# mitschabaude/msm-zprize

Measured on AMD Instinct MI355X. Metric: Mpoint-adds/s (ms per MSM in ms_per_step), higher is better.
Workload: dtype u32 limbs (28-bit lazy Montgomery, i64 accumulate)

## Files before the change

### msm_zprize_amd/_native.py

```python
import ctypes as C
import os

HERE = os.path.dirname(os.path.abspath(__file__))
LIB_PATH = os.environ.get("MSMZ_LIB") or os.path.join(HERE, "libmsmz.so")

MSMZ_N_STAGES = 8
STAGE_NAMES = ["digits", "scan", "scatter", "plan", "accumulate", "reduce", "final", "total"]


class MsmzOpts(C.Structure):
    _fields_ = [("c", C.c_int32), ("glv", C.c_int32), ("safe", C.c_int32), ("buckets", C.c_int32),
                ("timing", C.c_int32), ("reserved", C.c_int32 * 3)]


class MsmzLog(C.Structure):
    _fields_ = [("stage_ms", C.c_float * MSMZ_N_STAGES), ("c", C.c_int32), ("K", C.c_int32), ("rounds", C.c_int32),
                ("glv", C.c_int32), ("n_entries", C.c_uint64), ("n_pairs", C.c_uint64), ("max_bucket", C.c_uint32),
                ("scatter_launches", C.c_uint32), ("scatter_kernel_ms", C.c_float), ("batch_add_ms", C.c_float * 32)]


MSMZ_SRC_DEVICE, MSMZ_SRC_MONTGOMERY, MSMZ_SRC_DEFAULT_STREAM = 1, 2, 4
MSMZ_SRC_COMPRESSED, MSMZ_SRC_SIGN_PARITY = 8, 16
MSMZ_ERR_POINT = 7

# ... 76 lines not shown
                ("bins", C.c_void_p), ("packed", C.c_void_p)]


TEST_SORT_GEOM = ["c", "K", "Keff", "L", "nb", "fb", "fbt", "ncb", "ncbt", "nbins", "sbins", "fbins", "fine_top", "spread",
                  "fold_shift", "fold_rows", "F", "mbits", "idx_bits", "cspec", "two_level", "tiles", "sbits", "endo_delta"]


EXPORTS = {
    "msmz_create": (C.c_int, [C.POINTER(C.c_void_p), C.c_int, C.POINTER(C.c_int), C.c_int]),
    "msmz_destroy": (None, [C.c_void_p]),
    "msmz_strerror": (C.c_char_p, [C.c_int]),
    "msmz_curve_fe_bytes": (C.c_int, [C.c_int]),
    "msmz_ctx_fe_bytes": (C.c_int, [C.c_void_p]),
    "msmz_ctx_n_devices": (C.c_int, [C.c_void_p]),
    "msmz_upload_points": (C.c_int, [C.c_void_p, C.c_char_p, C.c_char_p, C.c_uint64, C.POINTER(C.c_uint64)]),
    "msmz_upload_scalars": (C.c_int, [C.c_void_p, C.c_char_p, C.c_uint64, C.POINTER(C.c_uint64)]),
    "msmz_import_scalars": (C.c_int, [C.c_void_p, C.POINTER(MsmzSrc), C.c_uint64, C.POINTER(C.c_uint64)]),
    "msmz_import_scalars_into": (C.c_int, [C.c_void_p, C.c_uint64, C.c_uint64, C.POINTER(MsmzSrc), C.c_uint64]),
    "msmz_alloc_scalars": (C.c_int, [C.c_void_p, C.c_uint64, C.POINTER(C.c_uint64)]),
    "msmz_import_points": (C.c_int, [C.c_void_p, C.POINTER(MsmzSrc), C.c_uint64, C.POINTER(C.c_uint64)]),
    "msmz_random_points": (C.c_int, [C.c_void_p, C.c_uint64, C.c_uint64, C.POINTER(C.c_uint64)]),
    "msmz_random_scalars": (C.c_int, [C.c_void_p, C.c_uint64, C.c_uint64, C.POINTER(C.c_uint64)]),
    "msmz_download_points": (C.c_int, [C.c_void_p, C.c_uint64, C.c_uint64, C.c_uint64, C.c_char_p, C.c_char_p]),
    "msmz_download_points_compressed": (C.c_int, [C.c_void_p, C.c_uint64, C.c_uint64, C.c_uint64, C.c_char_p, C.c_char_p,
                                                  C.c_uint32]),
    "msmz_download_scalars": (C.c_int, [C.c_void_p, C.c_uint64, C.c_uint64, C.c_uint64, C.c_char_p]),
    "msmz_free": (C.c_int, [C.c_void_p, C.c_uint64]),
    "msmz_msm": (C.c_int, [C.c_void_p, C.c_uint64, C.c_char_p, C.c_uint64, C.POINTER(MsmzOpts), C.c_char_p,
                           C.POINTER(C.c_int), C.POINTER(MsmzLog)]),
    "msmz_msm_resident": (C.c_int, [C.c_void_p, C.c_uint64, C.c_uint64, C.c_uint64, C.POINTER(MsmzOpts), C.c_char_p,
                                    C.POINTER(C.c_int), C.POINTER(MsmzLog)]),
    "msmz_msm_batch": (C.c_int, [C.c_void_p, C.c_uint64, C.c_char_p, C.c_uint64, C.c_uint32, C.POINTER(MsmzOpts),
                                 C.c_char_p, C.POINTER(C.c_int), C.POINTER(MsmzLog)]),
    "msmz_msm_batch_resident": (C.c_int, [C.c_void_p, C.c_uint64, C.c_uint64, C.c_uint64, C.c_uint32,
                                          C.POINTER(MsmzOpts), C.c_char_p, C.POINTER(C.c_int), C.POINTER(MsmzLog)]),
    "msmz_msm_segments": (C.c_int, [C.c_void_p, C.c_uint64, C.c_uint64, C.POINTER(MsmzSegment), C.c_uint32,
                                    C.POINTER(MsmzOpts), C.c_char_p, C.POINTER(C.c_int), C.POINTER(MsmzLog)]),
    "msmz_precompute_points": (C.c_int, [C.c_void_p, C.c_uint64, C.c_uint64, C.POINTER(MsmzOpts), C.c_uint32,
                                         C.POINTER(C.c_uint64)]),
    "msmz_precomputed_info": (C.c_int, [C.c_void_p, C.c_uint64, C.POINTER(C.c_int32), C.POINTER(C.c_int32),
                                        C.POINTER(C.c_uint32), C.POINTER(C.c_uint32), C.POINTER(C.c_uint64)]),
    "msmz_precomputed_scalar_bits": (C.c_int, [C.c_void_p, C.c_uint64, C.POINTER(C.c_int32)]),
    "msmz_check_points": (C.c_int, [C.c_void_p, C.c_uint64, C.c_uint64, C.c_uint64, C.c_uint32,
                                    C.POINTER(MsmzCheckResult), C.c_char_p]),
    "msmz_points_mul": (C.c_int, [C.c_void_p, C.POINTER(MsmzMul), C.c_uint64, C.POINTER(C.c_uint64)]),
    "msmz_points_mul_opts": (C.c_int, [C.c_void_p, C.POINTER(MsmzMul), C.c_uint64, C.POINTER(MsmzMulOpts),
                                       C.POINTER(C.c_uint64)]),
    "msmz_scalars_combine": (C.c_int, [C.c_void_p, C.POINTER(MsmzScalarTerm), C.POINTER(MsmzScalarTerm), C.c_uint64,
                                       C.c_uint64, C.POINTER(C.c_uint64)]),
    "msmz_scalars_dot": (C.c_int, [C.c_void_p, C.c_uint64, C.c_uint64, C.c_uint64, C.c_uint64, C.c_uint64, C.c_char_p]),
    "msmz_scalars_powers": (C.c_int, [C.c_void_p, C.c_char_p, C.c_char_p, C.c_uint64, C.POINTER(C.c_uint64)]),
    "msmz_scalars_recurrence": (C.c_int, [C.c_void_p, C.POINTER(MsmzScalarRec), C.c_uint64, C.c_uint64,
                                          C.POINTER(C.c_uint64), C.c_char_p]),
    "msmz_scalars_inverse": (C.c_int, [C.c_void_p, C.c_uint64, C.c_uint64, C.c_uint64, C.c_uint64, C.POINTER(C.c_uint64),
                                       C.POINTER(C.c_uint64)]),
    "msmz_scalars_ntt": (C.c_int, [C.c_void_p, C.POINTER(MsmzNtt), C.c_uint64, C.POINTER(C.c_uint64)]),
    "msmz_scalars_root_of_unity": (C.c_int, [C.c_int, C.c_uint32, C.c_char_p]),
    "msmz_point_add": (C.c_int, [C.c_int, C.c_char_p, C.c_int, C.c_char_p, C.c_int, C.c_char_p, C.POINTER(C.c_int)]),
    "msmz_test_set_glv_bits": (C.c_int, [C.c_void_p, C.c_int]),
    "msmz_test_retries": (C.c_int, [C.c_void_p]),
    "msmz_test_set_limits": (C.c_int, [C.c_void_p, C.c_uint64, C.c_uint64]),
    "msmz_test_passes": (C.c_int, [C.c_void_p, C.POINTER(C.c_uint64), C.POINTER(C.c_uint64)]),
    "msmz_test_scalar_dot_geometry": (None, [C.POINTER(C.c_uint32), C.POINTER(C.c_uint32)]),
    "msmz_test_scalar_scan_geometry": (None, [C.POINTER(C.c_uint32), C.POINTER(C.c_uint32), C.POINTER(C.c_uint32)]),
    "msmz_test_ntt_plan": (C.c_int, [C.c_int, C.c_uint32, C.POINTER(C.c_uint32), C.POINTER(C.c_uint32)]),
    "msmz_test_ntt_geometry": (None, [C.POINTER(C.c_uint32)]),
    "msmz_test_field": (C.c_int, [C.c_void_p, C.c_int, C.c_char_p, C.c_char_p, C.c_uint64, C.c_char_p]),
    "msmz_test_field_limbs": (C.c_int, [C.c_void_p, C.c_int, C.c_void_p, C.c_void_p, C.c_uint64, C.c_void_p,
                                        C.c_char_p]),
    "msmz_test_field_rows": (C.c_int, [C.c_void_p, C.c_int, C.c_void_p, C.c_void_p, C.c_uint64, C.c_uint32, C.c_void_p,
                                       C.c_char_p]),
    "msmz_test_glv": (C.c_int, [C.c_void_p, C.c_char_p, C.c_uint64, C.c_char_p, C.c_char_p, C.c_char_p]),
    "msmz_test_digits": (C.c_int, [C.c_void_p, C.c_char_p, C.c_uint64, C.c_int, C.c_int, C.c_int, C.c_void_p]),
    "msmz_test_sort": (C.c_int, [C.c_void_p, C.c_char_p, C.c_uint64, C.c_int, C.c_int, C.c_int, C.c_void_p, C.c_void_p,
                                 C.c_uint64, C.c_void_p, C.c_uint64]),
    "msmz_test_sort_ex": (C.c_int, [C.c_void_p, C.POINTER(MsmzTestSortArgs)]),
    "msmz_test_point_raw": (C.c_int, [C.c_void_p, C.c_int, C.c_char_p, C.c_char_p, C.c_char_p, C.c_uint64, C.c_int,
                                      C.c_char_p]),
    "msmz_test_point": (C.c_int, [C.c_void_p, C.c_int, C.c_char_p, C.c_char_p, C.c_char_p, C.c_char_p, C.c_uint64,
                                  C.c_char_p]),
    "msmz_test_batch_add": (C.c_int, [C.c_void_p, C.c_int, C.c_int, C.c_char_p, C.c_char_p, C.c_uint64, C.c_char_p,
                                      C.c_char_p, C.c_uint64, C.c_void_p, C.c_uint64, C.c_uint64, C.c_char_p,
                                      C.POINTER(C.c_uint32)]),
    "msmz_test_reduce": (C.c_int, [C.c_void_p, C.POINTER(MsmzTestReduceArgs)]),
    "msmz_test_plan": (C.c_int, [C.c_void_p, C.POINTER(MsmzTestPlanArgs)]),
}

_lib = None


class MsmzError(RuntimeError):
    def __init__(self, status, where):
        self.status = status
        msg = lib().msmz_strerror(status).decode() if _lib is not None else "?"
        super().__init__(f"{where}: msmz status {status} ({msg})")


def lib():
    global _lib
    if _lib is None:
        if not os.path.exists(LIB_PATH):
            raise RuntimeError(f"{LIB_PATH} is missing: run `python -m msm_zprize_amd.build` "
                               "(the MSM has no CPU fallback)")
        l = C.CDLL(LIB_PATH)
        for name, (res, args) in EXPORTS.items():
            fn = getattr(l, name)
            fn.restype = res
            fn.argtypes = args
        _lib = l
    return _lib


def check(status, where):
    if status != 0:
        raise MsmzError(status, where)
```

### msm_zprize_amd/csrc/batch_kernels.h

```cpp
#pragma once

namespace msmz {

#ifndef MSMZ_BATCH_BMAX
#define MSMZ_BATCH_BMAX 16
#endif
#ifdef MSMZ_EXP_NOMUL
#define BM_MUL(r, a, b) fe_add(r, a, b)
#define BM_SQR(r, a) fe_add(r, a, a)
#else
#define BM_MUL(r, a, b) fe_mul(r, a, b)
#define BM_SQR(r, a) fe_sqr(r, a)
#endif
enum { PK_NONE = 0, PK_ADD = 1, PK_DBL = 2, PK_TAKE_A = 3, PK_TAKE_B = 4, PK_INF = 5 };

template <class F, int T, bool SAFE, int OCC, int BMAX>
__global__ void __launch_bounds__(T, OCC) k_batch_add(uint32_t* slots, const uint32_t* points, const uint2* dsc,
                                                      uint32_t out_base, uint32_t total, int B, MsmMeta* meta) {
  __shared__ int32_t tree[F::N * T];
  __shared__ int32_t s_prev[F::N * T];
  __shared__ uint8_t s_kind[SAFE ? BMAX * T : 1];
  constexpr int N = F::N;
  const uint32_t block_base = blockIdx.x * (uint32_t)(T * B);
#ifdef MSMZ_TRACE
// ... 14 lines not shown
#pragma unroll 1
  for (int i = 0; i < B; i++) {
    const uint32_t t = block_base + (uint32_t)i * T + threadIdx.x;
    uint32_t kind = PK_NONE;
    uint2 dd = dnext;
    if (i + 1 < B && t + (uint32_t)T < total) dnext = dsc[t + (uint32_t)T];
    if (t < total) {
#if defined(MSMZ_EXP_LOCALMEM) || defined(MSMZ_EXP_LOCAL_FWD)
      dd.x = LOC_ORIG | (t & 4095u);
      dd.y = LOC_ORIG | ((t + 1u) & 4095u);
#endif
      Fe<F> d;
      kind = PK_ADD;
      if constexpr (SAFE && SlotFmt<F>::PACKED) {
        Fe<F> x1, x2;
        const uint32_t oa = load_operand_x_or<F>(x1, dd.x, slots, points);
        const uint32_t ob = load_operand_x_or<F>(x2, dd.y, slots, points);
        fe_sub(d, x2, x1);
        if (oa == 0 || ob == 0 || fe_is_zero(d)) {
          Affine<F> p1, p2;
          const bool infA = load_operand<F, true>(p1, dd.x, slots, points);
          const bool infB = load_operand<F, true>(p2, dd.y, slots, points);
          if (infA) {
            kind = infB ? PK_INF : PK_TAKE_B;
          } else if (infB) {
            kind = PK_TAKE_A;
          } else if (fe_is_zero(d)) {
            Fe<F> num;
            fe_sub(num, p2.y, p1.y);
            if (fe_is_zero(num) && !fe_is_zero(p1.y)) {
              kind = PK_DBL;
              fe_add(d, p2.y, p2.y);
            } else {
              kind = PK_INF;
            }
          }
        }
      } else if constexpr (SAFE) {
        Affine<F> p1, p2;
        const bool infA = load_operand<F, true>(p1, dd.x, slots, points);
        const bool infB = load_operand<F, true>(p2, dd.y, slots, points);
        Fe<F> num;
        fe_sub(d, p2.x, p1.x);
        fe_sub(num, p2.y, p1.y);
        if (infA) {
          kind = infB ? PK_INF : PK_TAKE_B;
        } else if (infB) {
          kind = PK_TAKE_A;
        } else if (fe_is_zero(d)) {
          if (fe_is_zero(num) && !fe_is_zero(p1.y)) {
            kind = PK_DBL;
            fe_add(d, p2.y, p2.y);
          } else {
            kind = PK_INF;
          }
        }
      } else {
        Fe<F> x1, x2;
        load_operand_x<F>(x1, dd.x, slots, points);
        load_operand_x<F>(x2, dd.y, slots, points);
        fe_sub(d, x2, x1);
      }
      if (kind == PK_ADD || kind == PK_DBL) {
        if (i == ilast) {
#pragma unroll
          for (int j = 0; j < N; j++) s_prev[j * T + threadIdx.x] = prefix.l[j];
        } else if (i > 0) {
#if defined(MSMZ_EXP_LOCALMEM) || defined(MSMZ_EXP_LOCAL_Z)
          slot_store_mulout<F>(slots + slot_offset<F>(blockIdx.x * 64u + (t & 63u)), prefix);
#else
          slot_store_mulout<F>(slots + slot_offset<F>(out_base + t), prefix);
#endif
        }
        Fe<F> np;
        BM_MUL(np, prefix, d);
        prefix = np;
      }
    }
    if (SAFE) s_kind[i * T + threadIdx.x] = (uint8_t)kind;
  }

  MSMZ_STAMP(trace, 1);
  __builtin_amdgcn_s_setprio(3);
  Fe<F> run;
  {
    Fe<F> partner, node;
#pragma unroll
    for (int j = 0; j < N; j++) partner.l[j] = __shfl_xor(prefix.l[j], 1, 64);
    fe_mul(node, prefix, partner);
    if ((threadIdx.x & 1) == 0) {
#pragma unroll
      for (int j = 0; j < N; j++) tree[j * T + (threadIdx.x >> 1)] = node.l[j];
    }
  }
  __syncthreads();
  int lvl_off = 0;
#pragma unroll 1
  for (int width = T >> 2; width >= 1; width >>= 1) {
    const int child_off = lvl_off;
    lvl_off += width * 2;
    if ((int)threadIdx.x < width) {
      Fe<F> x, y, z;
#pragma unroll
      for (int j = 0; j < N; j++) {
        x.l[j] = tree[j * T + child_off + 2 * threadIdx.x];
        y.l[j] = tree[j * T + child_off + 2 * threadIdx.x + 1];
      }
      fe_mul(z, x, y);
#pragma unroll
      for (int j = 0; j < N; j++) tree[j * T + lvl_off + threadIdx.x] = z.l[j];
    }
    __syncthreads();
  }
  MSMZ_STAMP(trace, 2);
  if (threadIdx.x < 64) {
    Fe<F> root, inv;
#pragma unroll
    for (int j = 0; j < N; j++) root.l[j] = tree[j * T + lvl_off];
#ifdef MSMZ_EXP_NOINV
    const bool ok = true;
    inv = root;
#else
    const bool ok = fe_inverse_wave(inv, root);
#endif
    if (threadIdx.x == 0) {
      if (!ok) atomicOr(&meta->error, 1u);
#pragma unroll
      for (int j = 0; j < N; j++) tree[j * T + lvl_off] = inv.l[j];
    }
  }
  __syncthreads();
  MSMZ_STAMP(trace, 3);
#pragma unroll 1
  for (int width = 1; width <= T >> 2; width <<= 1) {
    const int parent_off = lvl_off;
    lvl_off -= width * 2;
    Fe<F> ci;
    const bool mine = (int)threadIdx.x < 2 * width;
    if (mine) {
      Fe<F> pi, sib;
#pragma unroll
      for (int j = 0; j < N; j++) {
        pi.l[j] = tree[j * T + parent_off + (threadIdx.x >> 1)];
        sib.l[j] = tree[j * T + lvl_off + (threadIdx.x ^ 1)];
      }
      fe_mul(ci, pi, sib);
    }
    __syncthreads();
    if (mine) {
#pragma unroll
      for (int j = 0; j < N; j++) tree[j * T + lvl_off + threadIdx.x] = ci.l[j];
    }
    __syncthreads();
  }
  {
    Fe<F> partner, ninv;
#pragma unroll
    for (int j = 0; j < N; j++) {
      partner.l[j] = __shfl_xor(prefix.l[j], 1, 64);
      ninv.l[j] = tree[j * T + (threadIdx.x >> 1)];
    }
    fe_mul(run, ninv, partner);
  }

  MSMZ_STAMP(trace, 4);
  __builtin_amdgcn_s_setprio(0);
  {
    const uint32_t tl = block_base + (uint32_t)(B - 1) * T + threadIdx.x;
    if (tl < total) dnext = dsc[tl];
  }
#pragma unroll 1
  for (int i = B - 1; i >= 0; i--) {
    const uint32_t t = block_base + (uint32_t)i * T + threadIdx.x;
    uint2 dd = dnext;
    if (i > 0 && t - (uint32_t)T < total) dnext = dsc[t - (uint32_t)T];
    if (t >= total) continue;
    const uint32_t kind = SAFE ? s_kind[i * T + threadIdx.x] : (uint32_t)PK_ADD;
#if defined(MSMZ_EXP_LOCALMEM) || defined(MSMZ_EXP_LOCAL_BWD)
    dd.x = LOC_ORIG | (t & 4095u);
    dd.y = LOC_ORIG | ((t + 1u) & 4095u);
#endif
#if defined(MSMZ_EXP_LOCALMEM) || defined(MSMZ_EXP_LOCAL_Z)
    uint32_t* out = slots + slot_offset<F>(blockIdx.x * 64u + (t & 63u));
#else
    uint32_t* out = slots + slot_offset<F>(out_base + t);
#endif
    if (kind == PK_ADD || kind == PK_DBL) {
      Affine<F> p2;
      load_operand<F, false>(p2, dd.y, slots, points);
      Fe<F> z, mm, ms, d, tt, s12, num;
      if (i == ilast) {
#pragma unroll
        for (int j = 0; j < N; j++) z.l[j] = s_prev[j * T + threadIdx.x];
      } else if (i > 0) {
        slot_load_fe<F>(z, out);
      } else {
        fe_set_const<F>(z, F::ONE);
      }
      if (kind == PK_ADD) {
        Affine<F> p1;
        load_operand<F, false>(p1, dd.x, slots, points);
        fe_sub(d, p2.x, p1.x);
        fe_sub(num, p2.y, p1.y);
        fe_add(s12, p2.x, p1.x);
      } else {
        fe_add(d, p2.y, p2.y);
        fe_add(s12, p2.x, p2.x);
        Fe<F> xx;
        fe_sqr(xx, p2.x);
        fe_add(num, xx, xx);
        fe_add(num, num, xx);
        fe_carry(num);
      }
      BM_MUL(tt, z, run);
      BM_MUL(mm, num, tt);
      BM_MUL(tt, run, d);
      run = tt;
      BM_SQR(ms, mm);
      Affine<F> res;
      fe_sub(res.x, ms, s12);
      fe_sub(tt, p2.x, res.x);
      fe_carry(tt);
      BM_MUL(ms, mm, tt);
      fe_sub(res.y, ms, p2.y);
      slot_store_point<F>(out, res, false);
    } else if (kind == PK_TAKE_A || kind == PK_TAKE_B) {
      Affine<F> p;
      load_operand<F, false>(p, kind == PK_TAKE_A ? dd.x : dd.y, slots, points);
      slot_store_point<F>(out, p, false);
    } else {
      Affine<F> dummy;
      fe_zero(dummy.x);
      fe_zero(dummy.y);
      slot_store_point<F>(out, dummy, true);
    }
  }
  MSMZ_STAMP(trace, 5);
}

}
```

### msm_zprize_amd/csrc/instantiate.h

```cpp
#pragma once
#include "check_kernels.h"
#include "gen_kernels.h"
#include "import_kernels.h"
#include "kernels.h"
#include "mul_kernels.h"
#include "ntt_kernels.h"
#include "scalar_kernels.h"
#include "scan_kernels.h"
#include "test_kernels.h"

#if !defined(MSMZ_CURVE) || MSMZ_CURVE == 0
#define MSMZ_W0(X) X(Bls377Fp, Bls377Fr)
#else
#define MSMZ_W0(X)
#endif
#if !defined(MSMZ_CURVE) || MSMZ_CURVE == 1
#define MSMZ_W1(X) X(PallasFp, PallasFr)
#else
#define MSMZ_W1(X)
#endif
#if !defined(MSMZ_CURVE) || MSMZ_CURVE == 2
#define MSMZ_W2(X) X(Bls381Fp, Bls381Fr)
#else
#define MSMZ_W2(X)
// ... 33 lines not shown
                                                uint32_t, uint32_t);                                             \
  PFX template __global__ void k_pairsum<P>(uint32_t*, const uint32_t*, uint32_t);                               \
  PFX template __global__ void k_fill_neutral<P>(uint32_t*, uint32_t);                                           \
  PFX template __global__ void k_bucket_sums<P>(uint32_t*, const uint32_t*, const uint32_t*, uint32_t);          \
  PFX template __global__ void k_reduce2d_partial_acc<P>(uint32_t*, const uint32_t*, const uint32_t*, R2Geom, uint32_t); \
  PFX template __global__ void k_pairsum_x4<P>(uint32_t*, const uint32_t*, uint32_t);                            \
  PFX template __global__ void k_bucket_accumulate<P>(uint32_t*, const uint32_t*, const uint32_t*,               \
                                                      const uint32_t*, const uint32_t*, uint32_t, uint32_t, int);

#define MSMZ_INST_REDUCE(F, Fr, PFX)                                                                              \
  PFX template __global__ void k_reduce2d_partial<F>(uint32_t*, const uint32_t*, const uint32_t*, const uint4*,   \
                                                     R2Geom, uint32_t);                                          \
  PFX template __global__ void k_reduce_affine_finish<F>(uint32_t*, uint32_t*, const uint32_t*, const uint32_t*,  \
                                                         const uint2*, const uint4*, F2Geom);                     \
  MSMZ_INST_POLICY(WeierPolicy<F>, PFX)

#define MSMZ_INST_REDUCE_TE(F, Fr, PFX) MSMZ_INST_POLICY(TePolicy<F>, PFX)

#define MSMZ_INST_TEST(F, Fr, P, PFX)                                                                             \
  PFX template __global__ void k_test_field<F>(uint32_t*, const uint32_t*, const uint32_t*, uint32_t, int, uint32_t*); \
  PFX template __global__ void k_test_field_limbs<F>(int32_t*, uint32_t*, const int32_t*, const int32_t*, uint32_t,  \
                                                      int, uint32_t*);                                            \
  PFX template __global__ void k_test_field_rows<F>(int32_t*, uint32_t*, const int32_t*, const int32_t*, uint32_t,   \
                                                     int, uint32_t);                                              \
  PFX template __global__ void k_test_glv<Fr>(uint32_t*, uint32_t*, uint8_t*, const uint32_t*, uint32_t);         \
  PFX template __global__ void k_test_digits<Fr, false>(uint32_t*, const uint32_t*, uint32_t, int, int);          \
  PFX template __global__ void k_test_point<P>(uint32_t*, const uint32_t*, const uint32_t*, const uint8_t*,   \
                                                   const uint8_t*, uint32_t, int);                                \
  PFX template __global__ void k_test_point_raw<P>(uint32_t*, const uint32_t*, const uint32_t*, const uint8_t*, \
                                                       uint32_t, int, int);                                       \
  PFX template __global__ void k_test_accs_in<P>(uint32_t*, const uint32_t*, const uint8_t*, const uint32_t*, \
                                                     uint32_t, uint32_t*);                                        \
  PFX template __global__ void k_test_accs_out<P>(uint32_t*, const uint32_t*, uint32_t);

#define MSMZ_INST_SORT(Fr, PFX, GLV, C, SEG)                                                                      \
  PFX template __global__ void k_hist<Fr, GLV, C, SEG>(uint32_t*, uint16_t*, uint32_t*, MsmMeta*, const uint32_t*, SortGeom, uint32_t, const SegDesc*); \
  PFX template __global__ void k_coarse<Fr, GLV, C, SEG>(uint32_t*, const uint32_t*, const uint32_t*, const uint16_t*, const uint32_t*, SortGeom, uint32_t, const SegDesc*);

#define MSMZ_INST_SCAN(Fr, AM, HB, PFX)                                                                           \
  PFX template __global__ void k_scalars_rec_tile<Fr, AM, HB>(uint32_t*, uint32_t*, const uint32_t*, const uint32_t*, FrConst, uint32_t, uint32_t, uint32_t*); \
  PFX template __global__ void k_scalars_rec_apply<Fr, AM, HB>(uint32_t*, const uint32_t*, const uint32_t*, FrConst, const uint32_t*, uint32_t, uint32_t);

#define MSMZ_INST_SCALAR(Fr, PFX)                                                                                 \
  PFX template __global__ void k_digits<Fr, false>(uint32_t*, uint32_t*, MsmMeta*, const uint32_t*, uint32_t, int, int, int, int); \
  MSMZ_SORT_INSTANCES(MSMZ_INST_SORT, Fr, PFX)                                                                    \
  PFX template __global__ void k_check_scalars<Fr>(uint32_t*, const uint32_t*, uint32_t);                         \
  PFX template __global__ void k_gen_scalars<Fr>(uint32_t*, uint32_t, uint64_t, GenMap);                          \
  PFX template __global__ void k_import_scalars<Fr>(uint32_t*, const uint8_t*, uint64_t, int, uint32_t, int, uint32_t*); \
  PFX template __global__ void k_scalars_combine<Fr>(uint32_t*, ScalarTerm, ScalarTerm, uint32_t, uint32_t*);     \
  PFX template __global__ void k_scalars_dot<Fr>(uint32_t*, const uint32_t*, const uint32_t*, uint32_t, uint32_t*); \
  PFX template __global__ void k_scalars_dot_fold<Fr>(uint32_t*, const uint32_t*, uint32_t, int);                 \
  PFX template __global__ void k_scalars_powers<Fr>(uint32_t*, FrConst, FrPowTable, uint32_t, GenMap);                \
  MSMZ_INST_SCAN(Fr, SREC_A_NONE, true, PFX)                                                                      \
  MSMZ_INST_SCAN(Fr, SREC_A_BROADCAST, false, PFX)                                                                \
  MSMZ_INST_SCAN(Fr, SREC_A_BROADCAST, true, PFX)                                                                 \
  MSMZ_INST_SCAN(Fr, SREC_A_RESIDENT, false, PFX)                                                                 \
  MSMZ_INST_SCAN(Fr, SREC_A_RESIDENT, true, PFX)                                                                  \
  PFX template __global__ void k_scalars_rec_carry<Fr, false, true>(uint32_t*, uint32_t*, const uint32_t*, const uint32_t*, FrConst, uint32_t); \
  PFX template __global__ void k_scalars_rec_carry<Fr, true, false>(uint32_t*, uint32_t*, const uint32_t*, const uint32_t*, FrConst, uint32_t); \
  PFX template __global__ void k_scalars_rec_carry<Fr, true, true>(uint32_t*, uint32_t*, const uint32_t*, const uint32_t*, FrConst, uint32_t); \
  PFX template __global__ void k_scalars_inverse<Fr>(uint32_t*, const uint32_t*, uint32_t, uint32_t*);         \
  PFX template __global__ void k_ntt_pass<Fr>(NttArgs);

#define MSMZ_INST_MISC_P(F, Fr, P, PFX)                                                                           \
  PFX template __global__ void k_points_to_resident<P>(uint32_t*, const uint32_t*, const uint8_t*, uint32_t, int, uint32_t*); \
  PFX template __global__ void k_points_from_resident<P>(uint32_t*, const uint32_t*, uint32_t);                   \
  PFX template __global__ void k_import_points<P>(uint32_t*, const uint8_t*, uint64_t, const uint8_t*, uint32_t, int, int, uint32_t*); \
  PFX template __global__ void k_import_points_compressed<P>(uint32_t*, const uint8_t*, uint64_t, const uint8_t*, uint32_t, int, int, uint32_t*); \
  PFX template __global__ void k_points_compress<P>(uint32_t*, uint8_t*, const uint32_t*, uint32_t, int);         \
  PFX template __global__ void k_check_curve<P>(uint8_t*, CheckResult*, const uint32_t*, uint32_t, uint32_t);     \
  PFX template __global__ void k_check_subgroup<P, Fr>(uint8_t*, CheckResult*, const uint32_t*, uint32_t, uint32_t); \
  PFX template __global__ void k_points_mul<P, Fr, false>(uint32_t*, const uint32_t*, const uint32_t*, MulScalar, const uint32_t*, uint32_t, int, int, uint32_t*); \
  PFX template __global__ void k_points_mul<P, Fr, true>(uint32_t*, const uint32_t*, const uint32_t*, MulScalar, const uint32_t*, uint32_t, int, int, uint32_t*); \
  MSMZ_INST_TEST(F, Fr, P, PFX)                                                                                   \
  MSMZ_INST_SCALAR(Fr, PFX)

#define MSMZ_INST_MISC(F, Fr, PFX)                                                                                \
  MSMZ_INST_MISC_P(F, Fr, WeierPolicy<F>, PFX)                                                                    \
  PFX template __global__ void k_precompute_copy<F>(uint32_t*, const uint32_t*, uint32_t, int, int);              \
  PFX template __global__ void k_points_mul_glv<WeierPolicy<F>, Fr>(uint32_t*, const uint32_t*, const uint32_t*, MulGlvScalar, const uint32_t*, uint32_t, int, int, uint32_t*); \
  PFX template __global__ void k_digits<Fr, true>(uint32_t*, uint32_t*, MsmMeta*, const uint32_t*, uint32_t, int, int, int, int); \
  MSMZ_SORT_INSTANCES_WEIERSTRASS(MSMZ_INST_SORT, Fr, PFX)                                                        \
  PFX template __global__ void k_test_digits<Fr, true>(uint32_t*, const uint32_t*, uint32_t, int, int);           \
  PFX template __global__ void k_test_slots_in<F>(uint32_t*, const uint32_t*, const uint8_t*, uint32_t, uint32_t*); \
  PFX template __global__ void k_test_slots_out<F>(uint32_t*, const uint32_t*, uint32_t, uint32_t);

#define MSMZ_INST_MISC_TE(F, Fr, PFX) MSMZ_INST_MISC_P(F, Fr, TePolicy<F>, PFX)

#define MSMZ_INST_GEN_P(P, PFX)                                                  \
  PFX template __global__ void k_gen_table<P>(uint32_t*, const uint32_t*);       \
  PFX template __global__ void k_gen_points<P>(uint32_t*, const uint32_t*, uint32_t, uint64_t, int, GenMap);
#define MSMZ_INST_GEN(F, Fr, PFX) MSMZ_INST_GEN_P(WeierPolicy<F>, PFX)
#define MSMZ_INST_GEN_TE(F, Fr, PFX) MSMZ_INST_GEN_P(TePolicy<F>, PFX)

#define MSMZ_EXTERN extern
#define MSMZ_DEFINE
```

### msm_zprize_amd/csrc/kernels.h

```cpp
#pragma once
#include <hip/hip_runtime.h>
#include "constants_gen.h"
#include "plan.h"
#include "curve.h"
#include "fp_rows.h"
#include "scalar.h"

namespace msmz {

constexpr uint32_t REF_NEG = 0x80000000u;
constexpr uint32_t REF_IDX = 0x7fffffffu;

struct MsmMeta {
  uint32_t max_bucket;
  uint32_t n_entries;
  uint32_t error;
  uint32_t rounds;
  uint32_t round_pairs[32];
  uint32_t round_base[32];
};

typedef uint32_t u32x4 __attribute__((ext_vector_type(4)));

#ifndef MSMZ_POINT_PAD
// ... 334 lines not shown
      for (int i = 0; i < 2 * F::NW; i++) o |= w[i];
    }
    fe_unpack<F>(p.x, w);
    Fe<F> y;
    fe_unpack<F>(y, w + F::NW);
    fe_cneg(p.y, y, neg);
    return CHECK_INF && o == 0;
  } else {
    if (loc & LOC_ORIG) {
      uint32_t w[2 * F::NW];
      load_words<F>(w, points + (size_t)(loc & 0x3fffffffu) * PointFmt<F>::STRIDE);
      uint32_t o = 0;
      if (CHECK_INF) {
#pragma unroll
        for (int i = 0; i < 2 * F::NW; i++) o |= w[i];
      }
      fe_unpack<F>(p.x, w);
      Fe<F> y;
      fe_unpack<F>(y, w + F::NW);
      fe_cneg(p.y, y, loc >> 31);
      return CHECK_INF && o == 0;
    }
    return slot_load_point<F, CHECK_INF>(p, slots + slot_offset<F>(loc));
  }
}
template <class F>
__device__ __forceinline__ uint32_t load_operand_x_or(Fe<F>& x, uint32_t loc, const uint32_t* slots,
                                                      const uint32_t* points) {
  static_assert(SlotFmt<F>::PACKED, "packed slot records");
  int cs;
  uint32_t neg;
  const u32x4* s4 = reinterpret_cast<const u32x4*>(operand_address<F>(loc, slots, points, cs, neg));
  uint32_t w[F::NW];
  uint32_t o = 0;
#pragma unroll
  for (int i = 0; i < F::NW / 4; i++) {
    const u32x4 v = s4[i * cs];
    w[4 * i] = v.x;
    w[4 * i + 1] = v.y;
    w[4 * i + 2] = v.z;
    w[4 * i + 3] = v.w;
    o |= v.x | v.y | v.z | v.w;
  }
  fe_unpack<F>(x, w);
  return o;
}

template <class F>
__device__ __forceinline__ void load_operand_x(Fe<F>& x, uint32_t loc, const uint32_t* slots, const uint32_t* points) {
  if constexpr (SlotFmt<F>::PACKED) {
    int cs;
    uint32_t neg;
    const u32x4* s4 = reinterpret_cast<const u32x4*>(operand_address<F>(loc, slots, points, cs, neg));
    uint32_t w[F::NW];
#pragma unroll
    for (int i = 0; i < F::NW / 4; i++) {
      const u32x4 v = s4[i * cs];
      w[4 * i] = v.x;
      w[4 * i + 1] = v.y;
      w[4 * i + 2] = v.z;
      w[4 * i + 3] = v.w;
    }
    fe_unpack<F>(x, w);
  } else {
    if (loc & LOC_ORIG) {
      uint32_t w[F::NW];
      const u32x4* s4 = reinterpret_cast<const u32x4*>(points + (size_t)(loc & 0x3fffffffu) * PointFmt<F>::STRIDE);
#pragma unroll
      for (int i = 0; i < F::NW / 4; i++) {
        const u32x4 v = s4[i];
        w[4 * i] = v.x;
        w[4 * i + 1] = v.y;
        w[4 * i + 2] = v.z;
        w[4 * i + 3] = v.w;
      }
      fe_unpack<F>(x, w);
    } else {
      slot_load_fe<F>(x, slots + slot_offset<F>(loc));
    }
  }
}

template <class F>
__device__ __forceinline__ bool fe_inverse_wave(Fe<F>& r, const Fe<F>& x) {
  constexpr int N = F::N, W = F::W;
  constexpr uint32_t MASK = (1u << W) - 1u;
  static_assert(N <= 15, "one DPP row per vector");
  const int lane = (int)(threadIdx.x & 63u);
  const int row = lane >> 4, j = lane & 15;
  int32_t xl = 0, pl = 0, npl = 0;
  {
    Fe<F> xc;
    uint32_t w[F::NW];
    fe_to_canon_words<F>(w, x);
    fe_unpack<F>(xc, w);
#pragma unroll
    for (int k = 0; k < N; k++) {
      if (j == k) {
        xl = xc.l[k];
        pl = F::PL[k];
        npl = F::NPL[k];
      }
    }
  }
  int32_t val = row == 0 ? xl : row == 1 ? pl : (row == 2 && j == 0) ? 1 : 0;
  constexpr int ITERS = (2 * F::BITS + W - 1) / W + 1;
#pragma unroll 1
  for (int it = 0; it < ITERS; it++) {
    const uint64_t nz = __ballot(val != 0);
    const uint32_t ma = (uint32_t)nz & 0xffffu, mb = (uint32_t)(nz >> 16) & 0xffffu;
    if (ma == 0) break;
    const int h = 31 - __builtin_clz(ma | mb | 1u);
    const uint32_t a0 = (uint32_t)__builtin_amdgcn_readlane(val, 0), b0 = (uint32_t)__builtin_amdgcn_readlane(val, 16);
    uint64_t xa, xb;
    if (h == 0) {
      xa = a0;
      xb = b0;
    } else {
      const uint64_t ah = ((uint64_t)(uint32_t)__builtin_amdgcn_readlane(val, h) << W) |
                          (uint32_t)__builtin_amdgcn_readlane(val, h - 1);
      const uint64_t bh = ((uint64_t)(uint32_t)__builtin_amdgcn_readlane(val, 16 + h) << W) |
                          (uint32_t)__builtin_amdgcn_readlane(val, 16 + h - 1);
      if (h == 1) {
        xa = ah;
        xb = bh;
      } else {
        const uint64_t mx = ah | bh;
        const int len = 64 - __builtin_clzll(mx | 1);
        const int sh = len > (W + 1) ? len - (W + 1) : 0;
        xa = ((ah >> sh) << W) | (uint64_t)(a0 & MASK);
        xb = ((bh >> sh) << W) | (uint64_t)(b0 & MASK);
      }
    }
    int32_t f0 = 1, g0 = 0, f1 = 0, g1 = 1;
    int rem = W;
    while (true) {
      int tz = xa == 0 ? rem : __builtin_ctzll(xa);
      if (tz > rem) tz = rem;
      xa >>= tz;
      f1 <<= tz;
      g1 <<= tz;
      rem -= tz;
      if (rem == 0) break;
      if (xa < xb) {
        const uint64_t tx = xa; xa = xb; xb = tx;
        int32_t ti = f0; f0 = f1; f1 = ti;
        ti = g0; g0 = g1; g1 = ti;
      }
      xa -= xb;
      f0 -= f1;
      g0 -= g1;
    }
    const int32_t Fc = (row & 1) ? g1 : f0, Gc = (row & 1) ? f1 : g0;
    const int32_t partner = __shfl_xor(val, 16, 64);
    int64_t t = (int64_t)val * Fc + (int64_t)partner * Gc;
    uint32_t qu = (uint32_t)__builtin_amdgcn_readlane((int32_t)(uint32_t)t, 32);
    uint32_t qv = (uint32_t)__builtin_amdgcn_readlane((int32_t)(uint32_t)t, 48);
    if (F::PINV != 1u) {
      qu *= F::PINV;
      qv *= F::PINV;
    }
    const int32_t q = row == 2 ? (int32_t)(qu & MASK) : row == 3 ? (int32_t)(qv & MASK) : 0;
    t += (int64_t)q * npl;
    const int32_t lo = (int32_t)((uint32_t)t & MASK);
    const int32_t hi = (int32_t)(t >> W);
    val = __builtin_amdgcn_update_dpp(0, lo, 0x101, 0xf, 0xf, true) + hi;
    if (j >= N) val = 0;
    val = limb_row_ripple<W, N>(val, j);
    const int32_t top_u = __builtin_amdgcn_readlane(val, 32 + N - 1), top_v = __builtin_amdgcn_readlane(val, 48 + N - 1);
    if (row == 2 && top_u < 0) val += pl;
    if (row == 3 && top_v < 0) val += pl;
    const int32_t top_a = __builtin_amdgcn_readlane(val, N - 1), top_b = __builtin_amdgcn_readlane(val, 16 + N - 1);
    if ((top_a | top_b) < 0) {
      const bool neg = (row & 1) ? (top_b < 0) : (top_a < 0);
      val = neg ? -val : val;
      val = limb_row_ripple<W, N>(val, j);
    }
  }
  const uint64_t bad = __ballot(row == 1 && val != (j == 0 ? 1 : 0));
  if (bad != 0) {
    fe_zero(r);
    return false;
  }
  Fe<F> v, r3;
#pragma unroll
  for (int k = 0; k < N; k++) v.l[k] = __builtin_amdgcn_readlane(val, 48 + k);
  fe_carry(v);
  fe_set_const<F>(r3, F::R3);
  fe_mul<F>(r, v, r3);
  return true;
}

}

#include "batch_kernels.h"
#include "precompute_kernels.h"

namespace msmz {

template <class F>
__device__ __forceinline__ void fe_sel4(Fe<F>& r, int s, const Fe<F>& a0, const Fe<F>& a1, const Fe<F>& a2,
                                        const Fe<F>& a3) {
#pragma unroll
  for (int j = 0; j < F::N; j++) {
    int32_t lo = (s & 1) ? a1.l[j] : a0.l[j];
    int32_t hi = (s & 1) ? a3.l[j] : a2.l[j];
    r.l[j] = (s & 2) ? hi : lo;
  }
}

template <int J, class F>
__device__ __forceinline__ void fe_quad_bcast(Fe<F>& r, const Fe<F>& a) {
#pragma unroll
  for (int j = 0; j < F::N; j++) r.l[j] = __builtin_amdgcn_update_dpp(0, a.l[j], J * 0x55, 0xf, 0xf, false);
}

template <class F>
__device__ __forceinline__ void fe_pick(Fe<F>& r, bool c, const Fe<F>& a, const Fe<F>& b) {
#pragma unroll
  for (int j = 0; j < F::N; j++) r.l[j] = c ? a.l[j] : b.l[j];
}

template <class F>
__device__ __forceinline__ void xyzz_add_x4(Xyzz<F>& r, const Xyzz<F>& p, const Xyzz<F>& q, int s, bool dbl) {
  const bool pinf = xyzz_is_inf(p), qinf = xyzz_is_inf(q);
  Fe<F> a, b, m, U1, U2, S1, S2, P, R, PP, RR, Zm, Zc, PPP, Q, t, u, U, M, zero;
  fe_zero(zero);
  fe_sel4(a, s, p.X, q.X, p.Y, q.Y);
  fe_sel4(b, s, q.ZZ, p.ZZ, q.ZZZ, p.ZZZ);
  fe_mul(m, a, b);
  fe_quad_bcast<0>(U1, m);
  fe_quad_bcast<1>(U2, m);
  fe_quad_bcast<2>(S1, m);
  fe_quad_bcast<3>(S2, m);
  fe_sub(P, U2, U1);
  fe_sub(R, S2, S1);
  fe_add(U, p.Y, p.Y);
  fe_carry(U);
  fe_sel4(a, s, P, R, p.ZZ, p.ZZZ);
  fe_sel4(b, s, P, R, q.ZZ, q.ZZZ);
  fe_pick(t, (s & 1) != 0, p.X, U);
  fe_pick(a, dbl, t, a);
  fe_pick(b, dbl, t, b);
  fe_mul(m, a, b);
  fe_quad_bcast<0>(PP, m);
  fe_quad_bcast<1>(RR, m);
  fe_quad_bcast<2>(Zm, m);
  fe_quad_bcast<3>(Zc, m);
  fe_add(M, RR, RR);
  fe_add(M, M, RR);
  fe_carry(M);
  fe_sel4(a, s, P, U1, Zm, Zm);
  fe_sel4(t, s, U, p.X, M, p.ZZ);
  fe_pick(a, dbl, t, a);
  fe_pick(b, dbl && s == 2, M, PP);
  fe_mul(m, a, b);
  fe_quad_bcast<0>(PPP, m);
  fe_quad_bcast<1>(Q, m);
  fe_quad_bcast<2>(t, m);
  fe_quad_bcast<3>(u, m);
  fe_pick(r.ZZ, dbl, u, t);
  fe_pick(RR, dbl, t, RR);
  fe_pick(u, dbl, zero, PPP);
  fe_sub(t, RR, u);
  fe_sub(t, t, Q);
  fe_sub(u, t, Q);
  fe_carry(u);
  fe_sub(t, Q, u);
  fe_carry(t);
  fe_sel4(a, s, R, S1, Zc, Zc);
  fe_sel4(m, s, M, p.Y, p.ZZZ, p.ZZZ);
  fe_pick(a, dbl, m, a);
  fe_pick(b, s == 0, t, PPP);
  fe_mul(m, a, b);
  fe_quad_bcast<0>(Q, m);
  fe_quad_bcast<1>(t, m);
  fe_quad_bcast<2>(r.ZZZ, m);
// ... 564 lines not shown
```

### msm_zprize_amd/csrc/msmz.hip

```cpp
#include "instantiate.h"
namespace msmz {
#define X(F, Fr) MSMZ_INST_BATCH(F, Fr, MSMZ_EXTERN) MSMZ_INST_REDUCE(F, Fr, MSMZ_EXTERN) MSMZ_INST_MISC(F, Fr, MSMZ_EXTERN) MSMZ_INST_GEN(F, Fr, MSMZ_EXTERN)
MSMZ_WEIERSTRASS_FIELDS(X)
#undef X
#define X(F, Fr) MSMZ_INST_REDUCE_TE(F, Fr, MSMZ_EXTERN) MSMZ_INST_MISC_TE(F, Fr, MSMZ_EXTERN) MSMZ_INST_GEN_TE(F, Fr, MSMZ_EXTERN)
MSMZ_TE_FIELDS(X)
#undef X
}
#include "test_hooks.h"

namespace msmz {

template <class F_, class Fr_>
struct WeierCfg {
  using F = F_;
  using Fr = Fr_;
  using P = WeierPolicy<F>;
  static constexpr bool TE = false;
  static constexpr bool HAS_ENDO = true;
};

template <class F_, class Fr_>
struct TeCfg {
  using F = F_;
// ... 236 lines not shown
  }
}
int msmz_scalars_root_of_unity(int curve_id, uint32_t log_n, uint8_t* out_le32) {
  uint32_t w[8];
  const int S = ntt_two_adicity(curve_id, log_n, w);
  if (S < 0 || !out_le32) return MSMZ_ERR_ARG;
  if (log_n > (uint32_t)S) return MSMZ_ERR_UNSUPPORTED;
  memcpy(out_le32, w, 32);
  return MSMZ_OK;
}
int msmz_test_ntt_plan(int curve_id, uint32_t log_n, uint32_t* n_passes, uint32_t* stages) {
  const int S = ntt_two_adicity(curve_id, 0, nullptr);
  if (S < 0 || !n_passes || !stages || log_n > (uint32_t)NTT_MAX_LOG) return MSMZ_ERR_ARG;
  if (log_n > (uint32_t)S) return MSMZ_ERR_UNSUPPORTED;
  const NttPlan p = ntt_plan(log_n);
  *n_passes = p.n_passes;
  for (uint32_t j = 0; j < 8; j++) stages[j] = j < p.n_passes ? p.pass[j].s : 0;
  return MSMZ_OK;
}
void msmz_test_ntt_geometry(uint32_t* pass_log) {
  if (pass_log) *pass_log = NTT_PASS_LOG;
}
void msmz_test_scalar_dot_geometry(uint32_t* tile_elements, uint32_t* partials_per_pass) {
  if (tile_elements) *tile_elements = SDOT_TILE;
  if (partials_per_pass) *partials_per_pass = SDOT_PASS;
}
void msmz_test_scalar_scan_geometry(uint32_t* rec_tile, uint32_t* rec_pass, uint32_t* inv_chunk) {
  if (rec_tile) *rec_tile = SREC_TILE;
  if (rec_pass) *rec_pass = SREC_PASS;
  if (inv_chunk) *inv_chunk = SINV_CHUNK;
}

int msmz_test_set_glv_bits(msmz_ctx* c, int bits) { return c ? c->engine->test_set_glv_bits(bits) : MSMZ_ERR_ARG; }
int msmz_test_retries(msmz_ctx* c) { return c ? c->engine->test_retries() : -1; }
int msmz_test_set_limits(msmz_ctx* c, uint64_t pass_entries, uint64_t batch_entries) {
  return c ? c->engine->test_set_limits(pass_entries, batch_entries) : MSMZ_ERR_ARG;
}
int msmz_test_passes(msmz_ctx* c, uint64_t* range_passes, uint64_t* sub_batches) {
  if (!c) return MSMZ_ERR_ARG;
  c->engine->test_passes(range_passes, sub_batches);
  return MSMZ_OK;
}
int msmz_test_field(msmz_ctx* c, int op, const uint8_t* a, const uint8_t* b, uint64_t n, uint8_t* out) {
  return c ? c->engine->test_hooks()->test_field(op, a, b, n, out) : MSMZ_ERR_ARG;
}
int msmz_test_field_limbs(msmz_ctx* c, int op, const int32_t* a, const int32_t* b, uint64_t n, int32_t* raw,
                          uint8_t* canon) {
  return c ? c->engine->test_hooks()->test_field_limbs(op, a, b, n, raw, canon) : MSMZ_ERR_ARG;
}
int msmz_test_field_rows(msmz_ctx* c, int op, const int32_t* a, const int32_t* b, uint64_t n, uint32_t live_rows,
                         int32_t* raw, uint8_t* canon) {
  return c ? c->engine->test_hooks()->test_field_rows(op, a, b, n, live_rows, raw, canon) : MSMZ_ERR_ARG;
}
int msmz_test_glv(msmz_ctx* c, const uint8_t* s, uint64_t n, uint8_t* s0, uint8_t* s1, uint8_t* neg) {
  return c ? c->engine->test_hooks()->test_glv(s, n, s0, s1, neg) : MSMZ_ERR_ARG;
}
int msmz_test_digits(msmz_ctx* c, const uint8_t* s, uint64_t n, int cc, int K, int glv, uint32_t* digits) {
  return c ? c->engine->test_hooks()->test_digits(s, n, cc, K, glv, digits) : MSMZ_ERR_ARG;
}
int msmz_test_sort(msmz_ctx* c, const uint8_t* s, uint64_t n, int cc, int glv, int force_fallback, uint32_t* geom,
                   uint32_t* off, uint64_t off_cap, uint32_t* refs, uint64_t refs_cap) {
  if (!c) return MSMZ_ERR_ARG;
  return c->engine->test_hooks()->test_sort(s, n, cc, glv, force_fallback, geom, off, off_cap, refs, refs_cap);
}
int msmz_test_sort_ex(msmz_ctx* c, const msmz_test_sort_args* a) {
  return c && a ? c->engine->test_hooks()->test_sort_ex(*a) : MSMZ_ERR_ARG;
}
int msmz_test_point_raw(msmz_ctx* c, int op, const uint8_t* a, const uint8_t* b, const uint8_t* neg, uint64_t n, int L,
                        uint8_t* out) {
  return c ? c->engine->test_hooks()->test_point_raw(op, a, b, neg, n, L, out) : MSMZ_ERR_ARG;
}
int msmz_test_point(msmz_ctx* c, int op, const uint8_t* a, const uint8_t* ai, const uint8_t* b, const uint8_t* bi,
                    uint64_t n, uint8_t* out) {
  return c ? c->engine->test_hooks()->test_point(op, a, ai, b, bi, n, out) : MSMZ_ERR_ARG;
}

int msmz_test_batch_add(msmz_ctx* c, int safe, int B, const uint8_t* pxy, const uint8_t* pinf, uint64_t np,
                        const uint8_t* sxy, const uint8_t* sinf, uint64_t ns, const uint32_t* desc, uint64_t n_pairs,
                        uint64_t out_base, uint8_t* out, uint32_t* error) {
  if (!c) return MSMZ_ERR_ARG;
  return c->engine->test_hooks()->test_batch_add(safe, B, pxy, pinf, np, sxy, sinf, ns, desc, n_pairs, out_base, out, error);
}

int msmz_test_reduce(msmz_ctx* c, const msmz_test_reduce_args* a) {
  return c && a ? c->engine->test_hooks()->test_reduce(*a) : MSMZ_ERR_ARG;
}

int msmz_test_plan(msmz_ctx* c, const msmz_test_plan_args* a) {
  return c && a ? c->engine->test_hooks()->test_plan(*a) : MSMZ_ERR_ARG;
}

int msmz_point_add(int curve_id, const uint8_t* a, int ai, const uint8_t* b, int bi, uint8_t* out, int* oi) {
  if (!out || !oi || (!a && !ai) || (!b && !bi)) return MSMZ_ERR_ARG;
  switch (curve_id) {
    case MSMZ_BLS12_377_G1: return host_point_add<CfgBls377::P>(a, ai, b, bi, out, oi);
    case MSMZ_PALLAS: return host_point_add<CfgPallas::P>(a, ai, b, bi, out, oi);
    case MSMZ_BLS12_381_G1: return host_point_add<CfgBls381::P>(a, ai, b, bi, out, oi);
    case MSMZ_ED_ON_BLS12_377: return host_point_add<CfgEd377::P>(a, 0, b, 0, out, oi);
    default: return MSMZ_ERR_UNSUPPORTED;
  }
}

}
```

Measured before the change: 4802.

## Use row-parallel field multiplies for the upper levels of the batch-inverse tree

Moves the workgroup batch-inversion tree into its own helper. For large fields (N>9) on the unsafe path, the narrow upper levels now use a row-form multiply where each 16-lane row cooperates on one product, instead of leaving most threads idle. The top of the tree is reduced inside one wave using shuffles, and the inverse is computed in row form. This adds more barriers and row-form conversion overhead, and may not pay off if those levels were a small part of kernel time. A test hook for the batch inverse is also added.

```diff
diff --git a/msm_zprize_amd/_native.py b/msm_zprize_amd/_native.py
--- a/msm_zprize_amd/_native.py
+++ b/msm_zprize_amd/_native.py
@@ -182,6 +182,8 @@
     "msmz_test_batch_add": (C.c_int, [C.c_void_p, C.c_int, C.c_int, C.c_char_p, C.c_char_p, C.c_uint64, C.c_char_p,
                                       C.c_char_p, C.c_uint64, C.c_void_p, C.c_uint64, C.c_uint64, C.c_char_p,
                                       C.POINTER(C.c_uint32)]),
+    "msmz_test_batch_invert": (C.c_int, [C.c_void_p, C.c_int, C.c_void_p, C.c_uint32, C.c_uint32, C.c_void_p,
+                                         C.c_char_p, C.POINTER(C.c_uint32)]),
     "msmz_test_reduce": (C.c_int, [C.c_void_p, C.POINTER(MsmzTestReduceArgs)]),
     "msmz_test_plan": (C.c_int, [C.c_void_p, C.POINTER(MsmzTestPlanArgs)]),
 }
diff --git a/msm_zprize_amd/csrc/batch_invert.h b/msm_zprize_amd/csrc/batch_invert.h
--- /dev/null
+++ b/msm_zprize_amd/csrc/batch_invert.h
@@ -0,0 +1,189 @@
+#pragma once
+
+namespace msmz {
+
+#ifdef MSMZ_TRACE
+#define MSMZ_STAMP_OPT(tr, slot) do { if (tr) MSMZ_STAMP(tr, slot); } while (0)
+#else
+#define MSMZ_STAMP_OPT(tr, slot) do {} while (0)
+#endif
+
+#ifndef MSMZ_BATCH_ROW_W
+#define MSMZ_BATCH_ROW_W -1
+#endif
+template <class F, bool SAFE>
+constexpr int batch_row_w() {
+  if (MSMZ_BATCH_ROW_W >= 0) return MSMZ_BATCH_ROW_W;
+  return F::N > 9 && !SAFE ? 16 : 0;
+}
+
+template <class F, int I = 0>
+struct RowToFe {
+  static __device__ __forceinline__ void run(Fe<F>& r, int32_t x) {
+    r.l[I] = row_bcast<I>(x);
+    if constexpr (I + 1 < F::N) RowToFe<F, I + 1>::run(r, x);
+  }
+};
+
+template <class F, int T, int ROW_W>
+__device__ __forceinline__ Fe<F> wg_batch_inverse(const Fe<F>& prefix, int32_t* tree, MsmMeta* meta, uint64_t* trace) {
+  constexpr int N = F::N;
+  static_assert(ROW_W == 0 || ROW_W == 8 || ROW_W == 16 || ROW_W == 32, "row-form levels: 0, 8, 16 or 32 parents");
+  static_assert(T >= 64 && (T & (T - 1)) == 0, "whole waves, a full binary tree");
+  Fe<F> run;
+  {
+    Fe<F> partner, node;
+#pragma unroll
+    for (int j = 0; j < N; j++) partner.l[j] = __shfl_xor(prefix.l[j], 1, 64);
+    fe_mul(node, prefix, partner);
+    if ((threadIdx.x & 1) == 0) {
+#pragma unroll
+      for (int j = 0; j < N; j++) tree[j * T + (threadIdx.x >> 1)] = node.l[j];
+    }
+  }
+  __syncthreads();
+  int lvl_off = 0;
+  int width = T >> 2;
+#pragma unroll 1
+  for (; width > ROW_W && width >= 1; width >>= 1) {
+    const int child_off = lvl_off;
+    lvl_off += width * 2;
+    if ((int)threadIdx.x < width) {
+      Fe<F> x, y, z;
+#pragma unroll
+      for (int j = 0; j < N; j++) {
+        x.l[j] = tree[j * T + child_off + 2 * threadIdx.x];
+        y.l[j] = tree[j * T + child_off + 2 * threadIdx.x + 1];
+      }
+      fe_mul(z, x, y);
+#pragma unroll
+      for (int j = 0; j < N; j++) tree[j * T + lvl_off + threadIdx.x] = z.l[j];
+    }
+    __syncthreads();
+  }
+  if constexpr (ROW_W == 0) {
+    MSMZ_STAMP_OPT(trace, 2);
+    if (threadIdx.x < 64) {
+      Fe<F> root, inv;
+#pragma unroll
+      for (int j = 0; j < N; j++) root.l[j] = tree[j * T + lvl_off];
+#ifdef MSMZ_EXP_NOINV
+      const bool ok = true;
+      inv = root;
+#else
+      const bool ok = fe_inverse_wave(inv, root);
+#endif
+      if (threadIdx.x == 0) {
+        if (!ok) atomicOr(&meta->error, 1u);
+#pragma unroll
+        for (int j = 0; j < N; j++) tree[j * T + lvl_off] = inv.l[j];
+      }
+    }
+    __syncthreads();
+    MSMZ_STAMP_OPT(trace, 3);
+    width = 1;
+  } else {
+    const RowLane<F> rk = row_lane<F>();
+    const int wave = __builtin_amdgcn_readfirstlane((int)(threadIdx.x >> 6));
+    const int row = (int)(threadIdx.x >> 4) & 3;
+    const bool limb = rk.j < N;
+    int32_t* const col = tree + rk.j * T;
+#pragma unroll 1
+    for (; width >= 8; width >>= 1) {
+      const int child_off = lvl_off;
+      lvl_off += width * 2;
+#pragma unroll 1
+      for (int base = wave * 4; base < width; base += T / 16) {
+        const int node = base + row;
+        int32_t x = 0, y = 0;
+        if (limb) {
+          x = col[child_off + 2 * node];
+          y = col[child_off + 2 * node + 1];
+        }
+        const int32_t z = fe_mul_row<F>(x, y, rk);
+        if (limb) col[lvl_off + node] = z;
+      }
+      __syncthreads();
+    }
+    if (wave == 0) {
+      int32_t x = 0, y = 0;
+      if (limb) {
+        x = col[lvl_off + 2 * row];
+        y = col[lvl_off + 2 * row + 1];
+      }
+      const int32_t n4 = fe_mul_row<F>(x, y, rk);
+      const int32_t s4 = __shfl_xor(n4, 16, 64);
+      const int32_t n2 = fe_mul_row<F>(n4, s4, rk);
+      const int32_t s2 = __shfl_xor(n2, 32, 64);
+      const int32_t root = fe_mul_row<F>(n2, s2, rk);
+      MSMZ_STAMP_OPT(trace, 2);
+#ifdef MSMZ_EXP_NOINV
+      const bool ok = true;
+      const int32_t inv = root;
+#else
+      Fe<F> rootfe;
+      RowToFe<F>::run(rootfe, root);
+      int32_t inv;
+      const bool ok = fe_inverse_wave_row<F>(inv, rootfe, rk);
+#endif
+      if (threadIdx.x == 0 && !ok) atomicOr(&meta->error, 1u);
+      MSMZ_STAMP_OPT(trace, 3);
+      const int32_t i2 = fe_mul_row<F>(inv, s2, rk);
+      const int32_t i4 = fe_mul_row<F>(i2, s4, rk);
+      if (limb) col[lvl_off + 8 + row] = i4;
+    }
+    lvl_off += 8;
+    __syncthreads();
+#pragma unroll 1
+    for (width = 4; width <= ROW_W && width <= T >> 2; width <<= 1) {
+      const int parent_off = lvl_off;
+      lvl_off -= width * 2;
+#pragma unroll 1
+      for (int base = wave * 4; base < 2 * width; base += T / 16) {
+        const int c = base + row;
+        int32_t pi = 0, sib = 0;
+        if (limb) {
+          pi = col[parent_off + (c >> 1)];
+          sib = col[lvl_off + (c ^ 1)];
+        }
+        const int32_t ci = fe_mul_row<F>(pi, sib, rk);
+        if (limb) col[lvl_off + c] = ci;
+      }
+      __syncthreads();
+    }
+  }
+#pragma unroll 1
+  for (; width <= T >> 2; width <<= 1) {
+    const int parent_off = lvl_off;
+    lvl_off -= width * 2;
+    Fe<F> ci;
+    const bool mine = (int)threadIdx.x < 2 * width;
+    if (mine) {
+      Fe<F> pi, sib;
+#pragma unroll
+      for (int j = 0; j < N; j++) {
+        pi.l[j] = tree[j * T + parent_off + (threadIdx.x >> 1)];
+        sib.l[j] = tree[j * T + lvl_off + (threadIdx.x ^ 1)];
+      }
+      fe_mul(ci, pi, sib);
+    }
+    __syncthreads();
+    if (mine) {
+#pragma unroll
+      for (int j = 0; j < N; j++) tree[j * T + lvl_off + threadIdx.x] = ci.l[j];
+    }
+    __syncthreads();
+  }
+  {
+    Fe<F> partner, ninv;
+#pragma unroll
+    for (int j = 0; j < N; j++) {
+      partner.l[j] = __shfl_xor(prefix.l[j], 1, 64);
+      ninv.l[j] = tree[j * T + (threadIdx.x >> 1)];
+    }
+    fe_mul(run, ninv, partner);
+  }
+  return run;
+}
+
+}
diff --git a/msm_zprize_amd/csrc/batch_kernels.h b/msm_zprize_amd/csrc/batch_kernels.h
--- a/msm_zprize_amd/csrc/batch_kernels.h
+++ b/msm_zprize_amd/csrc/batch_kernels.h
@@ -120,86 +120,12 @@
 
   MSMZ_STAMP(trace, 1);
   __builtin_amdgcn_s_setprio(3);
-  Fe<F> run;
-  {
-    Fe<F> partner, node;
-#pragma unroll
-    for (int j = 0; j < N; j++) partner.l[j] = __shfl_xor(prefix.l[j], 1, 64);
-    fe_mul(node, prefix, partner);
-    if ((threadIdx.x & 1) == 0) {
-#pragma unroll
-      for (int j = 0; j < N; j++) tree[j * T + (threadIdx.x >> 1)] = node.l[j];
-    }
-  }
-  __syncthreads();
-  int lvl_off = 0;
-#pragma unroll 1
-  for (int width = T >> 2; width >= 1; width >>= 1) {
-    const int child_off = lvl_off;
-    lvl_off += width * 2;
-    if ((int)threadIdx.x < width) {
-      Fe<F> x, y, z;
-#pragma unroll
-      for (int j = 0; j < N; j++) {
-        x.l[j] = tree[j * T + child_off + 2 * threadIdx.x];
-        y.l[j] = tree[j * T + child_off + 2 * threadIdx.x + 1];
-      }
-      fe_mul(z, x, y);
-#pragma unroll
-      for (int j = 0; j < N; j++) tree[j * T + lvl_off + threadIdx.x] = z.l[j];
-    }
-    __syncthreads();
-  }
-  MSMZ_STAMP(trace, 2);
-  if (threadIdx.x < 64) {
-    Fe<F> root, inv;
-#pragma unroll
-    for (int j = 0; j < N; j++) root.l[j] = tree[j * T + lvl_off];
-#ifdef MSMZ_EXP_NOINV
-    const bool ok = true;
-    inv = root;
-#else
-    const bool ok = fe_inverse_wave(inv, root);
-#endif
-    if (threadIdx.x == 0) {
-      if (!ok) atomicOr(&meta->error, 1u);
-#pragma unroll
-      for (int j = 0; j < N; j++) tree[j * T + lvl_off] = inv.l[j];
-    }
-  }
-  __syncthreads();
-  MSMZ_STAMP(trace, 3);
-#pragma unroll 1
-  for (int width = 1; width <= T >> 2; width <<= 1) {
-    const int parent_off = lvl_off;
-    lvl_off -= width * 2;
-    Fe<F> ci;
-    const bool mine = (int)threadIdx.x < 2 * width;
-    if (mine) {
-      Fe<F> pi, sib;
-#pragma unroll
-      for (int j = 0; j < N; j++) {
-        pi.l[j] = tree[j * T + parent_off + (threadIdx.x >> 1)];
-        sib.l[j] = tree[j * T + lvl_off + (threadIdx.x ^ 1)];
-      }
-      fe_mul(ci, pi, sib);
-    }
-    __syncthreads();
-    if (mine) {
-#pragma unroll
-      for (int j = 0; j < N; j++) tree[j * T + lvl_off + threadIdx.x] = ci.l[j];
-    }
-    __syncthreads();
-  }
-  {
-    Fe<F> partner, ninv;
-#pragma unroll
-    for (int j = 0; j < N; j++) {
-      partner.l[j] = __shfl_xor(prefix.l[j], 1, 64);
-      ninv.l[j] = tree[j * T + (threadIdx.x >> 1)];
-    }
-    fe_mul(run, ninv, partner);
-  }
+#ifdef MSMZ_TRACE
+  uint64_t* const inv_trace = trace;
+#else
+  uint64_t* const inv_trace = nullptr;
+#endif
+  Fe<F> run = wg_batch_inverse<F, T, batch_row_w<F, SAFE>()>(prefix, tree, meta, inv_trace);
 
   MSMZ_STAMP(trace, 4);
   __builtin_amdgcn_s_setprio(0);
diff --git a/msm_zprize_amd/csrc/instantiate.h b/msm_zprize_amd/csrc/instantiate.h
--- a/msm_zprize_amd/csrc/instantiate.h
+++ b/msm_zprize_amd/csrc/instantiate.h
@@ -139,6 +139,8 @@
   PFX template __global__ void k_digits<Fr, true>(uint32_t*, uint32_t*, MsmMeta*, const uint32_t*, uint32_t, int, int, int, int); \
   MSMZ_SORT_INSTANCES_WEIERSTRASS(MSMZ_INST_SORT, Fr, PFX)                                                        \
   PFX template __global__ void k_test_digits<Fr, true>(uint32_t*, const uint32_t*, uint32_t, int, int);           \
+  PFX template __global__ void k_test_batch_invert<F, MSMZ_BATCH_T, false>(int32_t*, uint32_t*, uint32_t*, const int32_t*, uint32_t, MsmMeta*); \
+  PFX template __global__ void k_test_batch_invert<F, MSMZ_BATCH_T, true>(int32_t*, uint32_t*, uint32_t*, const int32_t*, uint32_t, MsmMeta*); \
   PFX template __global__ void k_test_slots_in<F>(uint32_t*, const uint32_t*, const uint8_t*, uint32_t, uint32_t*); \
   PFX template __global__ void k_test_slots_out<F>(uint32_t*, const uint32_t*, uint32_t, uint32_t);
 
diff --git a/msm_zprize_amd/csrc/kernels.h b/msm_zprize_amd/csrc/kernels.h
--- a/msm_zprize_amd/csrc/kernels.h
+++ b/msm_zprize_amd/csrc/kernels.h
@@ -440,7 +440,7 @@
 }
 
 template <class F>
-__device__ __forceinline__ bool fe_inverse_wave(Fe<F>& r, const Fe<F>& x) {
+__device__ __forceinline__ bool fe_inverse_wave_state(int32_t& val_out, const Fe<F>& x) {
   constexpr int N = F::N, W = F::W;
   constexpr uint32_t MASK = (1u << W) - 1u;
   static_assert(N <= 15, "one DPP row per vector");
@@ -535,8 +535,15 @@
       val = limb_row_ripple<W, N>(val, j);
     }
   }
-  const uint64_t bad = __ballot(row == 1 && val != (j == 0 ? 1 : 0));
-  if (bad != 0) {
+  val_out = val;
+  return __ballot(row == 1 && val != (j == 0 ? 1 : 0)) == 0;
+}
+
+template <class F>
+__device__ __forceinline__ bool fe_inverse_wave(Fe<F>& r, const Fe<F>& x) {
+  constexpr int N = F::N;
+  int32_t val;
+  if (!fe_inverse_wave_state<F>(val, x)) {
     fe_zero(r);
     return false;
   }
@@ -549,8 +556,21 @@
   return true;
 }
 
-}
-
+template <class F>
+__device__ __forceinline__ bool fe_inverse_wave_row(int32_t& r, const Fe<F>& x, const RowLane<F>& k) {
+  int32_t val;
+  if (!fe_inverse_wave_state<F>(val, x)) {
+    r = 0;
+    return false;
+  }
+  const int32_t v = fe_carry_row<F>(fe_from_row(val, 3), k);
+  r = fe_mul_row<F>(v, row_const<F>(F::R3, k.j), k);
+  return true;
+}
+
+}
+
+#include "batch_invert.h"
 #include "batch_kernels.h"
 #include "precompute_kernels.h"
 
diff --git a/msm_zprize_amd/csrc/msmz.hip b/msm_zprize_amd/csrc/msmz.hip
--- a/msm_zprize_amd/csrc/msmz.hip
+++ b/msm_zprize_amd/csrc/msmz.hip
@@ -342,6 +342,12 @@
   return c->engine->test_hooks()->test_batch_add(safe, B, pxy, pinf, np, sxy, sinf, ns, desc, n_pairs, out_base, out, error);
 }
 
+int msmz_test_batch_invert(msmz_ctx* c, int form, const int32_t* in_limbs, uint32_t n_groups, uint32_t n_live,
+                           int32_t* out_raw, uint8_t* out_canon, uint32_t* error) {
+  if (!c) return MSMZ_ERR_ARG;
+  return c->engine->test_hooks()->test_batch_invert(form, in_limbs, n_groups, n_live, out_raw, out_canon, error);
+}
+
 int msmz_test_reduce(msmz_ctx* c, const msmz_test_reduce_args* a) {
   return c && a ? c->engine->test_hooks()->test_reduce(*a) : MSMZ_ERR_ARG;
 }
```

Result: no change. 4836 (median of 6 runs) (+0.7%).
